# Vi-Sri/CerebralSignalNetworks

Measured on AMD Instinct MI355X. Metric: EEG-segments/sec training (128ch x 500, hidden=768), higher is better.
Workload: dtype bf16

## Files before the change

### cerebralsignalnetworks_amd/cabi.py

```python
import ctypes
import os

import torch

_HERE = os.path.dirname(os.path.abspath(__file__))
LIB_PATH = os.environ.get("CSN_LIB_PATH") or os.path.join(_HERE, "lib", "libcsn_hip.so")

CSN_F32, CSN_BF16 = 0, 1
STATUS_TIMEOUT, STATUS_NONFINITE, STATUS_STALE_SLOT = 1, 2, 4
ABI_VERSION = 6
LSTM_STATE = 0x100
LSTM_DROPOUT = 0x200
LSTM_REVERSE = 0x400
GRAD_OVERWRITE, GRAD_ACCUMULATE = 0, 1
SEG_DECAYED, SEG_SCALED = 1, 2

_c_void_p, _c_int, _c_i64, _c_size_t, _c_float = (ctypes.c_void_p, ctypes.c_int, ctypes.c_int64,
                                                  ctypes.c_size_t, ctypes.c_float)
_c_double = ctypes.c_double


class LstmDesc(ctypes.Structure):
    _fields_ = [("B", ctypes.c_int32), ("T", ctypes.c_int32), ("I", ctypes.c_int32),
                ("H", ctypes.c_int32), ("L", ctypes.c_int32), ("dtype", ctypes.c_int32)]
# ... 160 lines not shown
        _check(load().csn_eeg_bandpass_znorm(_ptr(x), B, C, T, sos.ctypes.data_as(ctypes.POINTER(ctypes.c_double)),
                                             sos.shape[0], int(ddof), _ptr(y), _dt(out_dtype), int(time_major), _stream()))
    return y


def _stream_rows(x_bct):
    B, C, T = x_bct.shape
    if not (x_bct.stride(2) == 1 and x_bct.stride(0) == C * x_bct.stride(1) and x_bct.stride(1) >= T):
        x_bct = x_bct.contiguous()
    return x_bct, x_bct.stride(1)


def _stream_state(t, name, shape, dtype):
    if t is None:
        return
    _need_cuda(t)
    if t.dtype != dtype or tuple(t.shape) != tuple(shape) or not t.is_contiguous():
        raise CsnError(f"eeg_bandpass_stream: {name} must be a contiguous {dtype} tensor of shape {tuple(shape)}, "
                       f"got {t.dtype} {tuple(t.shape)}")


def eeg_bandpass_stream(x_bct, sos, state_in=None, state_out=None, mean=None, inv_std=None, out_dtype=torch.float32,
                        time_major=False):
    import numpy as np
    _need_cuda(x_bct)
    if x_bct.dtype != torch.float32:
        raise CsnError("eeg_bandpass_stream expects float32 input")
    if x_bct.dim() != 3:
        raise CsnError(f"eeg_bandpass_stream expects x[B,C,T], got shape {tuple(x_bct.shape)}")
    x, row_stride = _stream_rows(x_bct)
    B, C, T = x.shape
    sos = np.ascontiguousarray(np.asarray(sos, dtype=np.float64).reshape(-1, 6)) if sos is not None else np.zeros((0, 6))
    nsec = sos.shape[0]
    if (mean is None) != (inv_std is None):
        raise CsnError("eeg_bandpass_stream: mean and inv_std are given together or not at all")
    _stream_state(state_in, "state_in", (B, C, nsec, 2), torch.float64)
    _stream_state(mean, "mean", (C,), torch.float32)
    _stream_state(inv_std, "inv_std", (C,), torch.float32)
    if state_out is None:
        state_out = torch.empty((B, C, nsec, 2), dtype=torch.float64, device=x.device)
    _stream_state(state_out, "state_out", (B, C, nsec, 2), torch.float64)
    y = torch.empty((T, B, C) if time_major else (B, T, C), dtype=out_dtype, device=x.device)
    with torch.cuda.device(x.device):
        _check(load().csn_eeg_bandpass_stream(_ptr(x), row_stride, B, C, T, sos.ctypes.data_as(ctypes.POINTER(ctypes.c_double)),
                                              nsec, _ptr(state_in), _ptr(state_out), _ptr(mean), _ptr(inv_std), _ptr(y),
                                              _dt(out_dtype), int(time_major), _stream()))
    return y, state_out


def eeg_bandpass_stream_path(x_bct, nsec):
    x, row_stride = _stream_rows(x_bct)
    B, C, T = x.shape
    return load().csn_eeg_bandpass_stream_path(_ptr(x), row_stride, C, T, int(nsec))


def eeg_filtfilt(x_stc, sos):
    import numpy as np
    _need_cuda(x_stc)
    x = x_stc.float().contiguous()
    S, T, C = x.shape
    sos = np.ascontiguousarray(np.asarray(sos, dtype=np.float64).reshape(-1, 6))
    lib = load()
    scratch = torch.empty(max(1, lib.csn_eeg_filtfilt_scratch_bytes(S, T, C, sos.shape[0])), dtype=torch.uint8,
                          device=x.device)
    y = torch.empty_like(x)
    with torch.cuda.device(x.device):
        _check(lib.csn_eeg_filtfilt(_ptr(x), S, T, C, sos.ctypes.data_as(ctypes.POINTER(ctypes.c_double)), sos.shape[0],
                                    _ptr(y), _ptr(scratch), _stream()))
    return y


def gemm_nt(a, bt, bias=None, out_dtype=torch.float32, out=None, accumulate=False):
    _need_cuda(a, bt)
    a, bt = a.contiguous(), bt.contiguous()
    M, K = a.shape
    N = bt.shape[0]
    assert bt.shape[1] == K and a.dtype == bt.dtype
    c = out if out is not None else torch.empty((M, N), dtype=out_dtype, device=a.device)
    _check(load().csn_gemm_nt(_ptr(a), _ptr(bt), _ptr(bias), _ptr(c), M, N, K, _dt(a.dtype), _dt(c.dtype),
                              int(accumulate), _stream()))
    return c


def gemm_tn(a_km, b_kn):
    _need_cuda(a_km, b_kn)
    a, b = a_km.contiguous(), b_kn.contiguous()
    K, M = a.shape
    N = b.shape[1]
    assert b.shape[0] == K and a.dtype == b.dtype
    lib = load()
    scratch = torch.empty(max(1, lib.csn_gemm_tn_scratch_bytes(M, N, K)), dtype=torch.uint8, device=a.device)
    c = torch.empty((M, N), dtype=torch.float32, device=a.device)
    _check(lib.csn_gemm_tn(_ptr(a), _ptr(b), _ptr(c), M, N, K, _dt(a.dtype), _ptr(scratch), _stream()))
    return c


def lstm_cell_forward(h_prev, w_hh, xproj, c_prev, want_gates=True):
    _need_cuda(w_hh, xproj)
    B, G = xproj.shape
    H = G // 4
    dt = w_hh.dtype
    gates = torch.empty((B, G), dtype=dt, device=xproj.device) if want_gates else None
    c_out = torch.empty((B, H), dtype=torch.float32, device=xproj.device)
    h_out = torch.empty((B, H), dtype=dt, device=xproj.device)
    _check(load().csn_lstm_cell_forward(_ptr(h_prev), _ptr(w_hh), _ptr(xproj), G, _ptr(c_prev), _ptr(gates),
                                        _ptr(c_out), _ptr(h_out), B, H, _dt(dt), _stream()))
    return h_out, c_out, gates


def lstm_cell_backward(dgates_next, w_hh_t, dy, gates, c, c_prev, dc_carry):
    _need_cuda(gates, c, dc_carry)
    B, G = gates.shape
    H = G // 4
    out = torch.empty_like(gates)
    _check(load().csn_lstm_cell_backward(_ptr(dgates_next), _ptr(w_hh_t), _ptr(dy), H, _ptr(gates), _ptr(c),
                                         _ptr(c_prev), _ptr(dc_carry), _ptr(out), B, H, _dt(gates.dtype), _stream()))
    return out


def _ptr_array(tensors):
    arr = (ctypes.c_void_p * len(tensors))()
    for i, t in enumerate(tensors):
        arr[i] = t.data_ptr()
    return arr


class LstmPlan:

    def __init__(self, B, T, I, H, L, dtype, device, training=True, state=False, dropout=False, reverse=False):
        self.desc = LstmDesc(B, T, I, H, L, _dt(dtype))
        self.training = bool(training)
        self.state = bool(state)
        self.dropout = bool(dropout)
        self.reverse = bool(reverse)
        self._io = (0, 0, False)
        self._views = None
        self.device = torch.device(device)
        lib = load()
        handle = _c_void_p()
        with torch.cuda.device(self.device):
            _check(lib.csn_lstm_plan_create(ctypes.byref(self.desc), int(self.training) | (LSTM_STATE if self.state else 0) |
                                            (LSTM_DROPOUT if self.dropout else 0) | (LSTM_REVERSE if self.reverse else 0),
                                            ctypes.byref(handle)))
        self._plan = handle
        nbytes = lib.csn_lstm_plan_workspace_bytes(self._plan)
        self.workspace = torch.empty(nbytes + 256, dtype=torch.uint8, device=self.device)
        off = (-self.workspace.data_ptr()) % 256
        self._ws_ptr = ctypes.c_void_p(self.workspace.data_ptr() + off)
        self.busy = False
        with torch.cuda.device(self.device):
            _check(lib.csn_lstm_workspace_init(self._plan, self._ws_ptr, _stream()))

    def __del__(self):
        plan, self._plan = getattr(self, "_plan", None), None
        if plan and _lib is not None:
            _lib.csn_lstm_plan_destroy(plan)

    def key(self):
        d = self.desc
        return ((d.B, d.T, d.I, d.H, d.L, d.dtype, self.training) + ((True,) if self.state else ()) +
                (("dropout plan",) if self.dropout else ()) + (("reverse plan",) if self.reverse else ()))

    def path(self):
        return load().csn_lstm_plan_path(self._plan)

    def kernel_names(self):
# ... 416 lines not shown
```

### cerebralsignalnetworks_amd/csrc/csn_common.h

```cpp
#pragma once
#include <hip/hip_runtime.h>
#include <stdint.h>
#include <stdio.h>
#include <stdlib.h>
#include <atomic>
#include <string>

#include "../../include/csn_hip.h"

namespace csn {

typedef __bf16 bf16_t;
typedef __attribute__((ext_vector_type(8))) __bf16 bf16x8;
typedef __attribute__((ext_vector_type(4))) __bf16 bf16x4;
typedef __attribute__((ext_vector_type(4))) float f32x4;
typedef __attribute__((ext_vector_type(4))) short s16x4;

void set_error(const std::string& msg);
int fail(int status, const char* fmt, ...);

#define CSN_HIP_CHECK(expr)                                                              \
  do {                                                                                   \
    hipError_t _e = (expr);                                                              \
    if (_e != hipSuccess)                                                                \
      return ::csn::fail(CSN_ERR_HIP, "%s failed: %s (%s:%d)", #expr, hipGetErrorString(_e), \
                         __FILE__, __LINE__);                                            \
  } while (0)

#define CSN_LAUNCH_CHECK()                                                               \
  do {                                                                                   \
    hipError_t _e = hipGetLastError();                                                   \
    if (_e != hipSuccess)                                                                \
      return ::csn::fail(CSN_ERR_HIP, "kernel launch failed: %s (%s:%d)",                \
                         hipGetErrorString(_e), __FILE__, __LINE__);                     \
  } while (0)

#define CSN_REQUIRE(cond, ...)                                                           \
  do {                                                                                   \
    if (!(cond)) return ::csn::fail(CSN_ERR_INVALID_ARGUMENT, __VA_ARGS__);              \
  } while (0)

struct Options {
  bool cell_v1, no_persist, no_persist_bwd, persist_streams, no_xcd_local, no_rotate, no_fuse_x, no_beside,
      no_side_stream, fwd_ksplit, fwd_nsplit, fwd_flags, bwd_flags, dpoll_no_hint, fwd_hint, gemm_no_dma, gemm_no_256, gemm_generic, tn_no_tr, tn_no_stagger, filter_v1, tags_no_rearm, gemm_no_192, no_half_tiles;
  int chunk;
  int tn_stages;
};
static inline Options options_from_env() {
  auto on = [](const char* name) { return getenv(name) != nullptr; };
  auto num = [](const char* name, int dflt) {
    const char* e = getenv(name);
    return e ? atoi(e) : dflt;
  };
  Options o{};
  o.cell_v1 = on("CSN_CELL_V1");
  o.no_persist = on("CSN_NO_PERSIST");
  o.no_persist_bwd = on("CSN_NO_PERSIST_BWD");
  o.persist_streams = on("CSN_PERSIST_STREAMS");
  o.no_xcd_local = on("CSN_NO_XCD_LOCAL");
  o.no_rotate = on("CSN_NO_ROTATE");
  o.no_fuse_x = on("CSN_NO_FUSE_X");
  o.no_beside = on("CSN_NO_BESIDE");
  o.no_half_tiles = on("CSN_NO_HALF_TILES");
  o.no_side_stream = on("CSN_NO_SIDE_STREAM");
  o.fwd_ksplit = on("CSN_FWD_KSPLIT");
  o.fwd_nsplit = on("CSN_FWD_NSPLIT");
  o.fwd_flags = on("CSN_FWD_FLAGS");
  o.bwd_flags = on("CSN_BWD_FLAGS");
  o.dpoll_no_hint = on("CSN_DPOLL_NO_HINT");
  o.fwd_hint = on("CSN_FWD_HINT");
  o.tn_no_stagger = on("CSN_TN_NO_STAGGER");
  o.gemm_no_dma = on("CSN_GEMM_NO_DMA");
  o.gemm_no_256 = on("CSN_GEMM_NO_256");
  o.gemm_no_192 = on("CSN_GEMM_NO_192");
  o.gemm_generic = on("CSN_GEMM_GENERIC");
  o.tn_no_tr = on("CSN_TN_NO_TR");
  o.filter_v1 = on("CSN_FILTER_V1");
#ifdef CSN_SLAB_TAGS
  o.tags_no_rearm = on("CSN_TAGS_NO_REARM");
#endif
  o.chunk = num("CSN_LSTM_CHUNK", 32);
  if (o.chunk < 1) o.chunk = 1;
  o.tn_stages = num("CSN_TN_STAGES", 4);
  return o;
}

static inline hipStream_t as_stream(csnStream_t s) { return reinterpret_cast<hipStream_t>(s); }
template <auto Kernel>
static int ensure_dyn_lds(int bytes) {
  static std::atomic<unsigned> done{0u};
  int dev = 0;
  CSN_HIP_CHECK(hipGetDevice(&dev));
  const unsigned bit = 1u << (dev & 31);
  if ((done.load(std::memory_order_acquire) & bit) == 0u) {
    CSN_HIP_CHECK(hipFuncSetAttribute(reinterpret_cast<const void*>(Kernel), hipFuncAttributeMaxDynamicSharedMemorySize, bytes));
    done.fetch_or(bit, std::memory_order_release);
  }
  return CSN_OK;
}

static inline size_t align_up(size_t v, size_t a) { return (v + a - 1) / a * a; }
static inline size_t dtype_size(int dtype) { return dtype == CSN_BF16 ? 2 : 4; }

__device__ __forceinline__ float to_f32(float v) { return v; }
__device__ __forceinline__ float to_f32(bf16_t v) { return (float)v; }
template <typename T> __device__ __forceinline__ T from_f32(float v);
template <> __device__ __forceinline__ float from_f32<float>(float v) { return v; }
template <> __device__ __forceinline__ bf16_t from_f32<bf16_t>(float v) { return (bf16_t)v; }

__device__ __forceinline__ float sigmoid_f32(float x) { return 1.0f / (1.0f + expf(-x)); }
__device__ __forceinline__ float tanh_f32(float x) { return tanhf(x); }

struct CellFwdOne {
  const void* h_prev; const void* w_hh; const float* xproj; int64_t xproj_ld; const float* c_prev;
  void* gates_out; float* c_out; void* h_out;
};
struct CellFwdBatch { CellFwdOne p[4]; };
struct CellBwdOne {
  const void* dg_next; const void* w_hh_t; const float* dy; int64_t dy_ld; const void* gates; const float* c;
  const float* c_prev; float* dc_carry; void* dg_out;
};
struct CellBwdBatch { CellBwdOne p[4]; };
struct CellMask {
  const int* lengths;
  int t[4];
};
struct CellNoMask {};
template <bool MASK> struct CellMaskArg { typedef CellNoMask type; };
template <> struct CellMaskArg<true> { typedef CellMask type; };
int launch_cell_fwd_batch(const CellFwdBatch& b, int np, int B, int H, int dtype, hipStream_t st);
int launch_cell_bwd_batch(const CellBwdBatch& b, int np, int B, int H, int dtype, hipStream_t st,
                          const CellMask* mask = nullptr);

int launch_cast_strided(const float* src, int64_t s0, int64_t s1, int64_t n0, int64_t n1, int64_t n2,
                        void* dst, int dtype, hipStream_t st, const int* len = nullptr, int rev = 0,
                        const int* vrow = nullptr, const int* vt0 = nullptr);
int launch_transpose_cast(const float* src, int64_t R, int64_t C, void* dst, int dtype, hipStream_t st);
int launch_cast(const float* src, void* dst, int64_t n, int dtype, hipStream_t st);
int launch_upcast(const void* src, int dtype, float* dst, int64_t n, hipStream_t st);
int launch_add_vec(const float* a, const float* b, float* out, int64_t n, hipStream_t st);
int launch_reduce_slabs(const float* slabs, int64_t stride, int S, float* out, float* out2, int64_t n, int accumulate,
                        hipStream_t st);
size_t colsum_scratch_bytes(int64_t N);
int launch_colsum(const void* X, int64_t R, int64_t N, int dtype, float* out, float* out2, int accumulate, void* scratch,
                  hipStream_t st);
int colsum_chunks();
int launch_colsum_partial(const void* X, int64_t R, int64_t N, int dtype, void* scratch, hipStream_t st);
int launch_gemm_tn_slabs(const void* A, const void* B, float* slabs, int64_t M, int64_t N, int64_t K, int dtype,
                         hipStream_t st, int* S_out, float* colsum, int* colsum_done, const Options& opt);
int gemm_nt(const void* A, const void* Bt, const float* bias, void* C, int64_t M, int64_t N, int64_t K, int dtype,
            int out_dtype, int accumulate, hipStream_t st, const Options& opt);
size_t gemm_tn_scratch_bytes(int64_t M, int64_t N, int64_t K, const Options& opt);

}
```

### cerebralsignalnetworks_amd/csrc/gemm.hip

```cpp
#include "csn_common.h"
#include "lstm_cell_common.h"

namespace csn {

template <typename T>
__global__ void __launch_bounds__(256)
gemm_generic_kernel(const T* __restrict__ A, int64_t sam, int64_t sak, const T* __restrict__ Bm, int64_t sbk,
                    int64_t sbn, const float* __restrict__ bias, void* __restrict__ Cv, int64_t ldc, int64_t M,
                    int64_t N, int64_t K, int out_bf16, int accumulate, int64_t k_per_split, int64_t slab_stride) {
  __shared__ float As[16][64 + 1];
  __shared__ float Bs[16][64 + 1];
  const int tid = threadIdx.x, lane = tid & 63, wave = tid >> 6;
  const int wm = wave >> 1, wn = wave & 1;
  const int64_t m0 = (int64_t)blockIdx.y * 64, n0 = (int64_t)blockIdx.x * 64;
  const int64_t kbeg = (int64_t)blockIdx.z * k_per_split;
  const int64_t kend = (kbeg + k_per_split < K) ? kbeg + k_per_split : K;
  const bool a_kfast = (sak == 1), b_kfast = (sbk == 1);

  f32x4 acc[2][2];
#pragma unroll
  for (int i = 0; i < 2; ++i)
#pragma unroll
    for (int j = 0; j < 2; ++j) acc[i][j] = (f32x4){0.f, 0.f, 0.f, 0.f};

// ... 713 lines not shown
  const int nrot_ = (int)(lid % (unsigned)nk);
#else
  const int nrot_ = 0;
#endif
  auto kpos = [&](int kt) { const int k = kt + nrot_; return (int64_t)(k >= nk ? k - nk : k) * 64; };
  auto issue_a = [&](int kt) {
    char* a_s = smem + (kt % 3) * 32768;
#pragma unroll
    for (int i = 0; i < 4; ++i) glds16(a_src[i] + kpos(kt), a_s + (8 * i + wave) * 1024);
  };
  auto issue_b = [&](int kt) {
    char* b_s = smem + kBBase + (kt % 2) * kBStage;
#pragma unroll
    for (int i = 0; i < NBI; ++i) glds16(b_src[i] + kpos(kt), b_s + (8 * i + wave) * 1024);
  };

  const unsigned sw = (unsigned)((lane & 15) >> 1);
  const unsigned a_base = (unsigned)((wm * 64 + (lane & 15)) * 128) + ((((unsigned)lane >> 4) ^ sw) << 4);
  const unsigned b_base = kBBase + (unsigned)((wn * (BN / 2) + (lane & 15)) * 128) + ((((unsigned)lane >> 4) ^ sw) << 4);

  f32x4 acc[4][NBF];
#pragma unroll
  for (int i = 0; i < 4; ++i)
#pragma unroll
    for (int j = 0; j < NBF; ++j) acc[i][j] = (f32x4){0.f, 0.f, 0.f, 0.f};

  issue_a(0);
  issue_b(0);
  if (nk > 1) issue_a(1);
  for (int kt = 0; kt < nk; ++kt) {
    if (kt + 1 < nk) asm volatile("s_waitcnt vmcnt(4)" ::: "memory");
    else asm volatile("s_waitcnt vmcnt(0)" ::: "memory");
    __builtin_amdgcn_s_barrier();
    if (kt + 1 < nk) issue_b(kt + 1);
    if (kt + 2 < nk) issue_a(kt + 2);
    const unsigned sa = (unsigned)(kt % 3) * 32768u, sb = (unsigned)(kt % 2) * kBStage;
#pragma unroll
    for (int kk = 0; kk < 2; ++kk) {
      const unsigned xo = kk ? 64u : 0u;
      bf16x8 af[4], bfr[NBF];
#pragma unroll
      for (int j = 0; j < NBF; ++j) bfr[j] = lds_read_b128(((b_base ^ xo) + sb) + j * 2048u);
#pragma unroll
      for (int i = 0; i < 4; ++i) af[i] = lds_read_b128(((a_base ^ xo) + sa) + i * 2048u);
#pragma unroll
      for (int i = 0; i < 4; ++i) {
        if (i == 0) asm volatile("s_waitcnt lgkmcnt(3)" ::: "memory");
        else if (i == 1) asm volatile("s_waitcnt lgkmcnt(2)" ::: "memory");
        else if (i == 2) asm volatile("s_waitcnt lgkmcnt(1)" ::: "memory");
        else asm volatile("s_waitcnt lgkmcnt(0)" ::: "memory");
        __builtin_amdgcn_sched_barrier(0);
#pragma unroll
        for (int j = 0; j < NBF; ++j)
          acc[i][j] = __builtin_amdgcn_mfma_f32_16x16x32_bf16(bfr[j], af[i], acc[i][j], 0, 0, 0);
        __builtin_amdgcn_sched_barrier(0);
      }
    }
  }

#pragma unroll
  for (int i = 0; i < 4; ++i) {
    const int64_t m = m0 + wm * 64 + i * 16 + (lane & 15);
    if (m >= M) continue;
#pragma unroll
    for (int j = 0; j < NBF; ++j) {
      const int64_t n = n0 + wn * (BN / 2) + j * 16 + (lane >> 4) * 4;
      f32x4 v = acc[i][j];
      if (bias) v += *reinterpret_cast<const f32x4*>(bias + n);
#if defined(CSN_NT_ABL) && CSN_NT_ABL == 1
      if (v[0] == v[0]) continue;
#endif
      if constexpr (sizeof(OutT) == 4) {
        f32x4* dst = reinterpret_cast<f32x4*>((float*)C + m * N + n);
        if (accumulate) v += *dst;
        *dst = v;
      } else {
        *reinterpret_cast<bf16x4*>((bf16_t*)C + m * N + n) = (bf16x4){(bf16_t)v[0], (bf16_t)v[1], (bf16_t)v[2], (bf16_t)v[3]};
      }
    }
  }
  }
}

__device__ __forceinline__ int tn256_lds_off(int krow, int col) {
  const int sw = (krow & 3) | (((krow >> 3) & 1) << 2);
  return krow * 512 + ((((col >> 4) ^ sw) << 4) + (col & 15)) * 2;
}
__device__ __forceinline__ bf16x8 tn256_load_frag(const char* tile, int mbase, int lane) {
  const int g = lane >> 4, i = lane & 15, q = i >> 2, p = i & 3;
  union { s16x4 s[2]; bf16x8 b; } u;
  u.s[0] = __builtin_amdgcn_ds_read_tr16_b64_v4i16(
      (__attribute__((address_space(3))) s16x4*)(tile + tn256_lds_off(8 * g + q, mbase + 4 * p)));
  u.s[1] = __builtin_amdgcn_ds_read_tr16_b64_v4i16(
      (__attribute__((address_space(3))) s16x4*)(tile + tn256_lds_off(8 * g + 4 + q, mbase + 4 * p)));
  return u.b;
}

__device__ __forceinline__ bf16x8 tr_read_pair(unsigned addr) {
  union { s16x4 s[2]; bf16x8 b; } u;
  asm volatile("ds_read_b64_tr_b16 %0, %1" : "=v"(u.s[0]) : "v"(addr) : "memory");
  asm volatile("ds_read_b64_tr_b16 %0, %1 offset:2048" : "=v"(u.s[1]) : "v"(addr) : "memory");
  return u.b;
}

template <int NSTAGE, bool COLSUM>
__global__ void __launch_bounds__(512)
gemm_tn_256_kernel(const bf16_t* __restrict__ A, const bf16_t* __restrict__ Bm, float* __restrict__ slabs,
                   int64_t M, int64_t N, int64_t K, int64_t k_per_split, float* __restrict__ colsum) {
  extern __shared__ __attribute__((aligned(1024))) char smem[];
  const int tid = threadIdx.x, lane = tid & 63, wave = tid >> 6;
  const int wm = wave >> 2, wn = wave & 3;
  const unsigned ntn = (unsigned)((N + 255) / 256), ntm = (unsigned)((M + 255) / 256);
  const unsigned lid = xcd_remap(blockIdx.x, gridDim.x);
  const unsigned zsplit = lid / (ntm * ntn), rem = lid % (ntm * ntn);
  const int64_t m0 = (int64_t)(rem / ntn) * 256, n0 = (int64_t)(rem % ntn) * 256;
  const int64_t kbeg = (int64_t)zsplit * k_per_split;
  const int64_t kend = (kbeg + k_per_split < K) ? kbeg + k_per_split : K;
  const int nh = kend > kbeg ? (int)((kend - kbeg) / 32) : 0;

  const bf16_t* a_src[2];
  const bf16_t* b_src[2];
#pragma unroll
  for (int i = 0; i < 2; ++i) {
    const int kr = 2 * (8 * i + wave) + (lane >> 5);
    const int c = lane & 31;
    const int sw = (kr & 3) | (((kr >> 3) & 1) << 2);
    const int col = (((c >> 1) ^ sw) << 4) + (c & 1) * 8;
    int64_t am = m0 + col, bn = n0 + col;
    am = am + 8 <= M ? am : M - 8;
    bn = bn + 8 <= N ? bn : N - 8;
    a_src[i] = A + (kbeg + kr) * M + am;
    b_src[i] = Bm + (kbeg + kr) * N + bn;
  }
#if defined(CSN_TN_ROT)
  const int rot_ = nh > CSN_TN_ROT ? (int)(rem % (unsigned)(CSN_TN_ROT)) : 0;
#endif
  auto issue = [&](int h) {
    char* a_s = smem + (h % NSTAGE) * 32768;
    char* b_s = a_s + 16384;
#if defined(CSN_TN_ROT)
    const int hs_ = h + rot_;
    const int64_t hr = hs_ >= nh ? hs_ - nh : hs_;
#else
    const int64_t hr = h;
#endif
#pragma unroll
    for (int i = 0; i < 2; ++i) {
      glds16(a_src[i] + hr * 32 * M, a_s + (8 * i + wave) * 1024);
      glds16(b_src[i] + hr * 32 * N, b_s + (8 * i + wave) * 1024);
    }
  };

  f32x4 acc[8][4];
#pragma unroll
  for (int i = 0; i < 8; ++i)
#pragma unroll
    for (int j = 0; j < 4; ++j) acc[i][j] = (f32x4){0.f, 0.f, 0.f, 0.f};
  const int wn_s = __builtin_amdgcn_readfirstlane(wn);
  const bool do_colsum = COLSUM && colsum != nullptr && n0 == 0;
  const bf16x8 ones = {(bf16_t)1.0f, (bf16_t)1.0f, (bf16_t)1.0f, (bf16_t)1.0f, (bf16_t)1.0f, (bf16_t)1.0f, (bf16_t)1.0f, (bf16_t)1.0f};
  f32x4 acc_cs[2];
  acc_cs[0] = acc_cs[1] = (f32x4){0.f, 0.f, 0.f, 0.f};

  unsigned a_addr[8], b_addr[4];
  {
    const int g = lane >> 4, q = (lane & 15) >> 2, pp = lane & 3;
// ... 243 lines not shown
          if (j == NJ / 4 && 2 * i < NP && more) issue_piece(h + PF, 2 * i);
          if (j == (3 * NJ) / 4 && 2 * i + 1 < NP && more) issue_piece(h + PF, 2 * i + 1);
          __builtin_amdgcn_sched_barrier(0);
#endif
        }
        if constexpr (COLSUM)
          if (own_cs & (1u << i))
            asm volatile("v_mfma_f32_16x16x32_bf16 %0, %1, %2, %0" : "+v"(acc_cs[i]) : "v"(ones), "v"(af[i]));
        __builtin_amdgcn_sched_barrier(0);
      }
      asm volatile("s_waitcnt lgkmcnt(2)" ::: "memory");
      __builtin_amdgcn_sched_barrier(0);
#pragma unroll
      for (int j = 0; j < NJ; ++j) {
#pragma unroll
        for (int k = 0; k < 4; ++k) {
          acc[4 + k][j] = __builtin_amdgcn_mfma_f32_16x16x32_bf16(__builtin_bit_cast(bf16x8, bfr[j]), __builtin_bit_cast(bf16x8, af[4 + k]), acc[4 + k][j], 0, 0, 0);
          __builtin_amdgcn_sched_barrier(0);
          if (k == 0) {
            if (j == 0) af[3] = W4_READ_A(3, sbn);
            else bfr[j - 1] = W4_READ_B(j - 1, sbn);
          }
          if (k == 3 && j == NJ - 1) bfr[j] = W4_READ_B(j, sbn);
          __builtin_amdgcn_sched_barrier(0);
        }
        if constexpr (COLSUM)
          if (j < 4 && (own_cs & (16u << j)))
            asm volatile("v_mfma_f32_16x16x32_bf16 %0, %1, %2, %0" : "+v"(acc_cs[4 + j]) : "v"(ones), "v"(af[4 + j]));
        __builtin_amdgcn_sched_barrier(0);
      }
    }
    asm volatile("s_waitcnt lgkmcnt(0)" ::: "memory");
  }
#undef W4_READ_A
#undef W4_READ_B

  if (COLSUM && (lane >> 4) == 0) {
#pragma unroll
    for (int e = 0; e < 8; ++e) {
      const int64_t m = m0 + wm * 128 + e * 16 + (lane & 15);
      if ((own_cs & (1u << e)) && m < M) colsum[(int64_t)zsplit * M + m] = acc_cs[e][0];
    }
  }

  float* C = slabs + (int64_t)zsplit * M * N;
#pragma unroll
  for (int i = 0; i < 8; ++i) {
    const int64_t m = m0 + wm * 128 + i * 16 + (lane & 15);
    if (m >= M) continue;
#pragma unroll
    for (int j = 0; j < NJ; ++j) {
      const int64_t n = n0 + wn * (BN / 2) + j * 16 + (lane >> 4) * 4;
      if (n + 3 < N && (N & 3) == 0) {
        *reinterpret_cast<float4*>(C + m * N + n) = make_float4(acc[i][j][0], acc[i][j][1], acc[i][j][2], acc[i][j][3]);
      } else {
        for (int r = 0; r < 4; ++r)
          if (n + r < N) C[m * N + n + r] = acc[i][j][r];
      }
    }
  }
}

static int tn_splits(int64_t M, int64_t N, int64_t K) {
  const int64_t tiles = ((M + 127) / 128) * ((N + 127) / 128);
  int64_t s = (1024 + tiles - 1) / tiles;
  const int64_t max_by_k = (K + 511) / 512;
  if (s > max_by_k) s = max_by_k;
  if (s < 1) s = 1;
  if (s > 64) s = 64;
  return (int)s;
}
static bool tn_use_256(int64_t M, int64_t N, int64_t K, const Options& opt) {
  return M >= 256 && N >= 128 && K % 64 == 0 && K >= 8192 && !opt.gemm_no_dma && !opt.gemm_no_256;
}
static int tn_splits_256(int64_t M, int64_t N, int64_t K) {
  const int64_t tiles = ((M + 255) / 256) * ((N + 255) / 256);
  int64_t s = 256 / tiles;
  const int64_t max_by_k = K / 2048;
  if (s > max_by_k) s = max_by_k;
  if (s < 1) s = 1;
  if (s > 64) s = 64;
  return (int)s;
}

int gemm_nt(const void* A, const void* Bt, const float* bias, void* C, int64_t M, int64_t N, int64_t K, int dtype,
            int out_dtype, int accumulate, hipStream_t st, const Options& opt) {
  CSN_REQUIRE(A && Bt && C, "csn_gemm_nt: null pointer");
  CSN_REQUIRE(M > 0 && N > 0 && K > 0, "csn_gemm_nt: bad shape M=%lld N=%lld K=%lld", (long long)M, (long long)N,
              (long long)K);
  CSN_REQUIRE(dtype == CSN_F32 || dtype == CSN_BF16, "csn_gemm_nt: bad dtype %d", dtype);
  CSN_REQUIRE(out_dtype == CSN_F32 || out_dtype == CSN_BF16, "csn_gemm_nt: bad out_dtype %d", out_dtype);
  CSN_REQUIRE(!(accumulate && out_dtype != CSN_F32), "csn_gemm_nt: accumulate needs a float32 C");
  const bool fast = dtype == CSN_BF16 && (K % 8 == 0) && (N % 4 == 0) &&
                    ((reinterpret_cast<uintptr_t>(A) | reinterpret_cast<uintptr_t>(Bt) |
                      reinterpret_cast<uintptr_t>(C) | reinterpret_cast<uintptr_t>(bias)) & 15) == 0 &&
                    !opt.gemm_generic;
  if (!fast)
    return launch_generic(A, K, 1, Bt, 1, K, bias, C, N, M, N, K, dtype, out_dtype, accumulate, 1, 0, st);
  if (K % 64 == 0 && K >= 128 && M >= 256 && !opt.gemm_no_dma && !opt.gemm_no_256 && !opt.gemm_no_192) {
    auto fills = [&](int bn) {
      if (N % bn != 0) return false;
      const int64_t t = (N / bn) * ((M + 255) / 256), rounds = (t + 255) / 256;
      return t >= 256 && t * 10 >= rounds * 256 * 9;
    };
    const int bn = fills(256) ? 256 : (fills(192) ? 192 : 0);
    if (bn != 0) {
      const int lds = 3 * 32768 + 2 * bn * 128;
      dim3 gridw((unsigned)((N / bn) * ((M + 255) / 256)));
      if (bn == 256) {
        if (int rc = ensure_dyn_lds<&gemm_nt_wide_kernel<bf16_t, 256>>(lds)) return rc;
        if (int rc = ensure_dyn_lds<&gemm_nt_wide_kernel<float, 256>>(lds)) return rc;
        if (out_dtype == CSN_BF16)
          gemm_nt_wide_kernel<bf16_t, 256><<<gridw, 512, lds, st>>>((const bf16_t*)A, (const bf16_t*)Bt, bias, (bf16_t*)C, M, N, K, 0);
        else
          gemm_nt_wide_kernel<float, 256><<<gridw, 512, lds, st>>>((const bf16_t*)A, (const bf16_t*)Bt, bias, (float*)C, M, N, K, accumulate);
      } else {
        if (int rc = ensure_dyn_lds<&gemm_nt_wide_kernel<bf16_t, 192>>(lds)) return rc;
        if (int rc = ensure_dyn_lds<&gemm_nt_wide_kernel<float, 192>>(lds)) return rc;
        if (out_dtype == CSN_BF16)
          gemm_nt_wide_kernel<bf16_t, 192><<<gridw, 512, lds, st>>>((const bf16_t*)A, (const bf16_t*)Bt, bias, (bf16_t*)C, M, N, K, 0);
        else
          gemm_nt_wide_kernel<float, 192><<<gridw, 512, lds, st>>>((const bf16_t*)A, (const bf16_t*)Bt, bias, (float*)C, M, N, K, accumulate);
      }
      CSN_LAUNCH_CHECK();
      return CSN_OK;
    }
  }
  if (K % 64 == 0 && K >= 256 && M >= 256 && N >= 1024 && !opt.gemm_no_dma && !opt.gemm_no_256) {
    if (int rc = ensure_dyn_lds<&gemm_nt_256_kernel<bf16_t, 3>>(3 * 49152)) return rc;
    if (int rc = ensure_dyn_lds<&gemm_nt_256_kernel<float, 3>>(3 * 49152)) return rc;
    dim3 grid256((unsigned)(((N + 127) / 128) * ((M + 255) / 256)));
    if (out_dtype == CSN_BF16)
      gemm_nt_256_kernel<bf16_t, 3><<<grid256, 512, 3 * 49152, st>>>((const bf16_t*)A, (const bf16_t*)Bt, bias, (bf16_t*)C, M, N, K, 0);
    else
      gemm_nt_256_kernel<float, 3><<<grid256, 512, 3 * 49152, st>>>((const bf16_t*)A, (const bf16_t*)Bt, bias, (float*)C, M, N, K, accumulate);
    CSN_LAUNCH_CHECK();
    return CSN_OK;
  }
  dim3 grid((unsigned)(((N + 127) / 128) * ((M + 127) / 128)));
  if (K % 64 == 0 && !opt.gemm_no_dma) {
    if (int rc = ensure_dyn_lds<&gemm_nt_dma_kernel<bf16_t>>(98304)) return rc;
    if (int rc = ensure_dyn_lds<&gemm_nt_dma_kernel<float>>(98304)) return rc;
    if (out_dtype == CSN_BF16)
      gemm_nt_dma_kernel<bf16_t><<<grid, 256, 65536, st>>>((const bf16_t*)A, (const bf16_t*)Bt, bias, (bf16_t*)C, M, N, K, 0);
    else
      gemm_nt_dma_kernel<float><<<grid, 256, 65536, st>>>((const bf16_t*)A, (const bf16_t*)Bt, bias, (float*)C, M, N, K, accumulate);
    CSN_LAUNCH_CHECK();
    return CSN_OK;
  }
  if (out_dtype == CSN_BF16)
    gemm_nt_bf16_kernel<bf16_t, 1><<<grid, 256, 32768, st>>>((const bf16_t*)A, (const bf16_t*)Bt, bias, (bf16_t*)C, M, N, K, 0);
  else
    gemm_nt_bf16_kernel<float, 1><<<grid, 256, 32768, st>>>((const bf16_t*)A, (const bf16_t*)Bt, bias, (float*)C, M, N, K, accumulate);
  CSN_LAUNCH_CHECK();
  return CSN_OK;
}

}

using namespace csn;

extern "C" int csn_gemm_nt(const void* A, const void* Bt, const float* bias, void* C, int64_t M, int64_t N, int64_t K,
                           int dtype, int out_dtype, int accumulate, csnStream_t stream) {
  return gemm_nt(A, Bt, bias, C, M, N, K, dtype, out_dtype, accumulate, as_stream(stream), options_from_env());
}

namespace csn {
size_t gemm_tn_scratch_bytes(int64_t M, int64_t N, int64_t K, const Options& opt) {
  if (M <= 0 || N <= 0 || K <= 0) return 0;
  const int a = tn_splits(M, N, K), b = tn_use_256(M, N, K, opt) ? tn_splits_256(M, N, K) : 0;
  return (size_t)(a > b ? a : b) * (size_t)M * (size_t)N * sizeof(float);
}
}

extern "C" size_t csn_gemm_tn_scratch_bytes(int64_t M, int64_t N, int64_t K) {
  return gemm_tn_scratch_bytes(M, N, K, options_from_env());
}

namespace csn {
int launch_gemm_tn_slabs(const void* A, const void* B, float* slabs, int64_t M, int64_t N, int64_t K, int dtype,
                         hipStream_t st, int* S_out, float* colsum, int* colsum_done, const Options& opt) {
  if (colsum_done) *colsum_done = 0;
  const bool aligned16 = ((reinterpret_cast<uintptr_t>(A) | reinterpret_cast<uintptr_t>(B)) & 15) == 0;
  if (dtype == CSN_BF16 && (M % 8 == 0) && (N % 8 == 0) && aligned16 && tn_use_256(M, N, K, opt)) {
    const int S2 = tn_splits_256(M, N, K);
    int64_t kper2 = (K + S2 - 1) / S2;
    kper2 = (kper2 + 63) / 64 * 64;
    *S_out = S2;
    if (int rc = ensure_dyn_lds<&gemm_tn_256_kernel<5, false>>(5 * 32768)) return rc;
    if (int rc = ensure_dyn_lds<&gemm_tn_256_kernel<4, false>>(4 * 32768)) return rc;
    if (int rc = ensure_dyn_lds<&gemm_tn_256_kernel<3, false>>(3 * 32768)) return rc;
    if (int rc = ensure_dyn_lds<&gemm_tn_256_kernel<4, true>>(4 * 32768)) return rc;
    dim3 grid((unsigned)(((N + 255) / 256) * ((M + 255) / 256) * S2));
    const int nst = opt.tn_stages;
    const bf16_t* Ab = (const bf16_t*)A;
    const bf16_t* Bb = (const bf16_t*)B;
    if (!opt.tn_no_stagger && nst == 4) {
      constexpr int NS = CSN_TN_W4_NSTAGE, PF = CSN_TN_W4_PF;
      if (N <= 128) {
        constexpr int lds = NS * (16384 + 8192);
        if (int rc = ensure_dyn_lds<&gemm_tn_256w4_kernel<NS, PF, false, 128>>(lds)) return rc;
        if (int rc = ensure_dyn_lds<&gemm_tn_256w4_kernel<NS, PF, true, 128>>(lds)) return rc;
        if (colsum) gemm_tn_256w4_kernel<NS, PF, true, 128><<<grid, 256, lds, st>>>(Ab, Bb, slabs, M, N, K, kper2, colsum);
        else gemm_tn_256w4_kernel<NS, PF, false, 128><<<grid, 256, lds, st>>>(Ab, Bb, slabs, M, N, K, kper2, nullptr);
      } else {
        constexpr int lds = NS * 32768;
        if (int rc = ensure_dyn_lds<&gemm_tn_256w4_kernel<NS, PF, false, 256>>(lds)) return rc;
        if (int rc = ensure_dyn_lds<&gemm_tn_256w4_kernel<NS, PF, true, 256>>(lds)) return rc;
        if (colsum) gemm_tn_256w4_kernel<NS, PF, true, 256><<<grid, 256, lds, st>>>(Ab, Bb, slabs, M, N, K, kper2, colsum);
        else gemm_tn_256w4_kernel<NS, PF, false, 256><<<grid, 256, lds, st>>>(Ab, Bb, slabs, M, N, K, kper2, nullptr);
      }
    } else if (colsum) gemm_tn_256_kernel<4, true><<<grid, 512, 4 * 32768, st>>>(Ab, Bb, slabs, M, N, K, kper2, colsum);
    else if (nst == 3) gemm_tn_256_kernel<3, false><<<grid, 512, 3 * 32768, st>>>(Ab, Bb, slabs, M, N, K, kper2, nullptr);
    else if (nst == 5) gemm_tn_256_kernel<5, false><<<grid, 512, 5 * 32768, st>>>(Ab, Bb, slabs, M, N, K, kper2, nullptr);
    else gemm_tn_256_kernel<4, false><<<grid, 512, 4 * 32768, st>>>(Ab, Bb, slabs, M, N, K, kper2, nullptr);
    if (colsum && colsum_done) *colsum_done = 1;
    CSN_LAUNCH_CHECK();
    return CSN_OK;
  }
  const int S = tn_splits(M, N, K);
  int64_t kper = (K + S - 1) / S;
  kper = (kper + 63) / 64 * 64;
  *S_out = S;
  const bool fast = dtype == CSN_BF16 && (M % 8 == 0) && (N % 8 == 0) &&
                    ((reinterpret_cast<uintptr_t>(A) | reinterpret_cast<uintptr_t>(B)) & 15) == 0 &&
                    !opt.gemm_generic;
  if (fast) {
    dim3 grid((unsigned)(((N + 127) / 128) * ((M + 127) / 128) * S));
    if (opt.tn_no_tr)
      gemm_tn_bf16_kernel<false><<<grid, 256, 0, st>>>((const bf16_t*)A, (const bf16_t*)B, slabs, M, N, K, kper);
    else
      gemm_tn_bf16_kernel<true><<<grid, 256, 0, st>>>((const bf16_t*)A, (const bf16_t*)B, slabs, M, N, K, kper);
    CSN_LAUNCH_CHECK();
    return CSN_OK;
  }
  return launch_generic(A, 1, M, B, N, 1, nullptr, slabs, N, M, N, K, dtype, CSN_F32, 0, S, M * N, st);
}
}

extern "C" int csn_gemm_tn(const void* A, const void* B, float* C, int64_t M, int64_t N, int64_t K, int dtype,
                           void* scratch, csnStream_t stream) {
  CSN_REQUIRE(A && B && C && scratch, "csn_gemm_tn: null pointer");
  CSN_REQUIRE(M > 0 && N > 0 && K > 0, "csn_gemm_tn: bad shape");
  CSN_REQUIRE(dtype == CSN_F32 || dtype == CSN_BF16, "csn_gemm_tn: bad dtype %d", dtype);
  hipStream_t st = as_stream(stream);
  int S = 1;
  if (int rc = launch_gemm_tn_slabs(A, B, (float*)scratch, M, N, K, dtype, st, &S, nullptr, nullptr, options_from_env())) return rc;
  return launch_reduce_slabs((const float*)scratch, M * N, S, C, nullptr, M * N, 0, st);
}
```

Baseline: 27010.

## Add 4-wave 256x192 NT GEMM kernel with two workgroups per CU

Adds a new bf16 NT GEMM kernel for the 192-wide tile case that uses 256 threads (4 waves) with 128x96 per-wave tiles, an A ring buffer of depth 3 and a double-buffered B stage. It uses swizzled LDS, hand-scheduled ds_read and MFMA interleaving, and async global-to-LDS loads. LDS is capped at 80KB so two workgroups can fit per CU. The aim is better occupancy and overlap than the 512-thread wide kernel on the 192-column path. The cost is high register pressure from 48 accumulators per lane. It also requires 32-bit byte offsets, which is guarded by a fit check.

```diff
diff --git a/cerebralsignalnetworks_amd/cabi.py b/cerebralsignalnetworks_amd/cabi.py
--- a/cerebralsignalnetworks_amd/cabi.py
+++ b/cerebralsignalnetworks_amd/cabi.py
@@ -266,6 +266,18 @@
     return c
 
 
+def gemm_nt_w4_offsets_fit(M, N, K):
+    fn = load().csn_gemm_nt_w4_offsets_fit
+    fn.restype, fn.argtypes = _c_int, [_c_i64, _c_i64, _c_i64]
+    return bool(fn(M, N, K))
+
+
+def gemm_nt_w4_lds_bytes():
+    fn = load().csn_gemm_nt_w4_lds_bytes
+    fn.restype, fn.argtypes = _c_int, []
+    return int(fn())
+
+
 def gemm_tn(a_km, b_kn):
     _need_cuda(a_km, b_kn)
     a, b = a_km.contiguous(), b_kn.contiguous()
diff --git a/cerebralsignalnetworks_amd/csrc/csn_common.h b/cerebralsignalnetworks_amd/csrc/csn_common.h
--- a/cerebralsignalnetworks_amd/csrc/csn_common.h
+++ b/cerebralsignalnetworks_amd/csrc/csn_common.h
@@ -42,7 +42,7 @@
 
 struct Options {
   bool cell_v1, no_persist, no_persist_bwd, persist_streams, no_xcd_local, no_rotate, no_fuse_x, no_beside,
-      no_side_stream, fwd_ksplit, fwd_nsplit, fwd_flags, bwd_flags, dpoll_no_hint, fwd_hint, gemm_no_dma, gemm_no_256, gemm_generic, tn_no_tr, tn_no_stagger, filter_v1, tags_no_rearm, gemm_no_192, no_half_tiles;
+      no_side_stream, fwd_ksplit, fwd_nsplit, fwd_flags, bwd_flags, dpoll_no_hint, fwd_hint, gemm_no_dma, gemm_no_256, gemm_generic, tn_no_tr, tn_no_stagger, filter_v1, tags_no_rearm, gemm_no_192, no_half_tiles, nt_no_w4;
   int chunk;
   int tn_stages;
 };
@@ -73,6 +73,7 @@
   o.gemm_no_dma = on("CSN_GEMM_NO_DMA");
   o.gemm_no_256 = on("CSN_GEMM_NO_256");
   o.gemm_no_192 = on("CSN_GEMM_NO_192");
+  o.nt_no_w4 = on("CSN_NT_NO_W4");
   o.gemm_generic = on("CSN_GEMM_GENERIC");
   o.tn_no_tr = on("CSN_TN_NO_TR");
   o.filter_v1 = on("CSN_FILTER_V1");
diff --git a/cerebralsignalnetworks_amd/csrc/gemm.hip b/cerebralsignalnetworks_amd/csrc/gemm.hip
--- a/cerebralsignalnetworks_amd/csrc/gemm.hip
+++ b/cerebralsignalnetworks_amd/csrc/gemm.hip
@@ -819,6 +819,120 @@
   }
 }
 
+#ifndef CSN_NT_W4_NA
+#define CSN_NT_W4_NA 3
+#endif
+__device__ __forceinline__ int nt64_sw(int row) {
+  const int g = (row >> 2) & 3;
+  return (((g ^ (g >> 1)) & 1) << 1) | (g >> 1);
+}
+template <typename OutT, int NA>
+__global__ void __launch_bounds__(256, 2)
+gemm_nt_w4_kernel(const bf16_t* __restrict__ A, const bf16_t* __restrict__ Bt, const float* __restrict__ bias,
+                  OutT* __restrict__ C, int64_t M, int64_t N, int64_t K, int accumulate) {
+  static_assert(NA == 2 || NA == 3, "A ring depth");
+  constexpr unsigned kAStage = 16384u, kBStage = 12288u, kBBase = NA * kAStage;
+  static_assert(kBBase + 2 * kBStage <= 81920u, "two workgroups per CU");
+  extern __shared__ __attribute__((aligned(1024))) char smem[];
+  const int tid = threadIdx.x, lane = tid & 63;
+  const int wave = __builtin_amdgcn_readfirstlane(tid >> 6);
+  const int wm = wave >> 1, wn = wave & 1;
+  const unsigned ntn = (unsigned)(N / 192);
+  const unsigned lid = xcd_remap(blockIdx.x, gridDim.x);
+  const int64_t m0 = (int64_t)(lid / ntn) * 256, n0 = (int64_t)(lid % ntn) * 192;
+  const int nk = __builtin_amdgcn_readfirstlane((int)(K / 32));
+
+  unsigned a_off[4], b_off[3];
+#pragma unroll
+  for (int i = 0; i < 4; ++i) {
+    const int row = (4 * i + wave) * 16 + (lane >> 2);
+    const int ch = (lane & 3) ^ nt64_sw(row);
+    int64_t am = m0 + row;
+    am = am < M ? am : M - 1;
+    a_off[i] = (unsigned)((am * K + ch * 8) * 2);
+  }
+#pragma unroll
+  for (int i = 0; i < 3; ++i) {
+    const int row = (4 * i + wave) * 16 + (lane >> 2);
+    const int ch = (lane & 3) ^ nt64_sw(row);
+    b_off[i] = (unsigned)(((n0 + row) * K + ch * 8) * 2);
+  }
+  auto issue_a = [&](int kt, int i) {
+    glds16(reinterpret_cast<const char*>(A + (int64_t)kt * 32) + a_off[i], smem + (unsigned)(kt % NA) * kAStage + (4 * i + wave) * 1024);
+  };
+  auto issue_b = [&](int kt, int i) {
+    glds16(reinterpret_cast<const char*>(Bt + (int64_t)kt * 32) + b_off[i], smem + kBBase + (unsigned)(kt & 1) * kBStage + (4 * i + wave) * 1024);
+  };
+
+  const unsigned frag = (unsigned)((lane & 15) * 64) + ((((unsigned)lane >> 4) ^ (unsigned)nt64_sw(lane & 15)) << 4);
+  const unsigned a_base = (unsigned)(wm * 128 * 64) + frag;
+  const unsigned b_base = kBBase + (unsigned)(wn * 96 * 64) + frag;
+#define W4_READ(addr, off) ({ bf16x8 v_; asm volatile("ds_read_b128 %0, %1 offset:%2" : "=v"(v_) : "v"(addr), "n"(off) : "memory"); v_; })
+
+  f32x4 acc[8][6];
+#pragma unroll
+  for (int i = 0; i < 8; ++i)
+#pragma unroll
+    for (int j = 0; j < 6; ++j) acc[i][j] = (f32x4){0.f, 0.f, 0.f, 0.f};
+
+#pragma unroll
+  for (int i = 0; i < 4; ++i) issue_a(0, i);
+#pragma unroll
+  for (int i = 0; i < 3; ++i) issue_b(0, i);
+  if (NA == 3 && nk > 1) {
+#pragma unroll
+    for (int i = 0; i < 4; ++i) issue_a(1, i);
+  }
+  for (int kt = 0; kt < nk; ++kt) {
+    if (NA == 3 && kt + 1 < nk) asm volatile("s_waitcnt vmcnt(4)" ::: "memory");
+    else asm volatile("s_waitcnt vmcnt(0)" ::: "memory");
+    __builtin_amdgcn_s_barrier();
+    const bool more_b = kt + 1 < nk, more_a = kt + NA - 1 < nk;
+    const unsigned aa = a_base + (unsigned)(kt % NA) * kAStage, ba = b_base + (unsigned)(kt & 1) * kBStage;
+    bf16x8 af[2], bfr[6];
+#pragma unroll
+    for (int j = 0; j < 6; ++j) bfr[j] = W4_READ(ba, j * 1024);
+    af[0] = W4_READ(aa, 0);
+#pragma unroll
+    for (int i = 0; i < 8; ++i) {
+      if (i < 7) af[(i + 1) & 1] = W4_READ(aa, (i + 1) * 1024);
+      if (i < 7) asm volatile("s_waitcnt lgkmcnt(1)" ::: "memory");
+      else asm volatile("s_waitcnt lgkmcnt(0)" ::: "memory");
+      __builtin_amdgcn_sched_barrier(0);
+#pragma unroll
+      for (int j = 0; j < 6; ++j) {
+        acc[i][j] = __builtin_amdgcn_mfma_f32_16x16x32_bf16(bfr[j], af[i & 1], acc[i][j], 0, 0, 0);
+        __builtin_amdgcn_sched_barrier(0);
+        if (j == 1) {
+          if (i < 3) { if (more_b) issue_b(kt + 1, i); }
+          else if (i < 7) { if (more_a) issue_a(kt + NA - 1, i - 3); }
+          __builtin_amdgcn_sched_barrier(0);
+        }
+      }
+    }
+  }
+#undef W4_READ
+
+#pragma unroll
+  for (int i = 0; i < 8; ++i) {
+    const int64_t m = m0 + wm * 128 + i * 16 + (lane & 15);
+    if (m >= M) continue;
+#pragma unroll
+    for (int j = 0; j < 6; ++j) {
+      const int64_t n = n0 + wn * 96 + j * 16 + (lane >> 4) * 4;
+      f32x4 v = acc[i][j];
+      if (bias) v += *reinterpret_cast<const f32x4*>(bias + n);
+      if constexpr (sizeof(OutT) == 4) {
+        f32x4* dst = reinterpret_cast<f32x4*>((float*)C + m * N + n);
+        if (accumulate) v += *dst;
+        *dst = v;
+      } else {
+        *reinterpret_cast<bf16x4*>((bf16_t*)C + m * N + n) = (bf16x4){(bf16_t)v[0], (bf16_t)v[1], (bf16_t)v[2], (bf16_t)v[3]};
+      }
+    }
+  }
+}
+
 __device__ __forceinline__ int tn256_lds_off(int krow, int col) {
   const int sw = (krow & 3) | (((krow >> 3) & 1) << 2);
   return krow * 512 + ((((col >> 4) ^ sw) << 4) + (col & 15)) * 2;
@@ -1228,6 +1342,13 @@
   if (s > 64) s = 64;
   return (int)s;
 }
+
+static bool nt_w4_offsets_fit(int64_t M, int64_t N, int64_t K) {
+  const int64_t lim = (int64_t)1 << 31;
+  return M <= lim / K && N <= lim / K && M * K < lim && N * K < lim;
+}
+static constexpr int kNtW4LdsBytes = CSN_NT_W4_NA * 16384 + 2 * 12288;
+static_assert(kNtW4LdsBytes <= 81920, "two workgroups of gemm_nt_w4_kernel per CU");
 
 int gemm_nt(const void* A, const void* Bt, const float* bias, void* C, int64_t M, int64_t N, int64_t K, int dtype,
             int out_dtype, int accumulate, hipStream_t st, const Options& opt) {
@@ -1260,6 +1381,13 @@
           gemm_nt_wide_kernel<bf16_t, 256><<<gridw, 512, lds, st>>>((const bf16_t*)A, (const bf16_t*)Bt, bias, (bf16_t*)C, M, N, K, 0);
         else
           gemm_nt_wide_kernel<float, 256><<<gridw, 512, lds, st>>>((const bf16_t*)A, (const bf16_t*)Bt, bias, (float*)C, M, N, K, accumulate);
+      } else if (!opt.nt_no_w4 && nt_w4_offsets_fit(M, N, K)) {
+        if (int rc = ensure_dyn_lds<&gemm_nt_w4_kernel<bf16_t, CSN_NT_W4_NA>>(kNtW4LdsBytes)) return rc;
+        if (int rc = ensure_dyn_lds<&gemm_nt_w4_kernel<float, CSN_NT_W4_NA>>(kNtW4LdsBytes)) return rc;
+        if (out_dtype == CSN_BF16)
+          gemm_nt_w4_kernel<bf16_t, CSN_NT_W4_NA><<<gridw, 256, kNtW4LdsBytes, st>>>((const bf16_t*)A, (const bf16_t*)Bt, bias, (bf16_t*)C, M, N, K, 0);
+        else
+          gemm_nt_w4_kernel<float, CSN_NT_W4_NA><<<gridw, 256, kNtW4LdsBytes, st>>>((const bf16_t*)A, (const bf16_t*)Bt, bias, (float*)C, M, N, K, accumulate);
       } else {
         if (int rc = ensure_dyn_lds<&gemm_nt_wide_kernel<bf16_t, 192>>(lds)) return rc;
         if (int rc = ensure_dyn_lds<&gemm_nt_wide_kernel<float, 192>>(lds)) return rc;
@@ -1318,6 +1446,11 @@
   return (size_t)(a > b ? a : b) * (size_t)M * (size_t)N * sizeof(float);
 }
 }
+
+extern "C" int csn_gemm_nt_w4_offsets_fit(int64_t M, int64_t N, int64_t K) {
+  return M > 0 && N > 0 && K > 0 && nt_w4_offsets_fit(M, N, K) ? 1 : 0;
+}
+extern "C" int csn_gemm_nt_w4_lds_bytes(void) { return kNtW4LdsBytes; }
 
 extern "C" size_t csn_gemm_tn_scratch_bytes(int64_t M, int64_t N, int64_t K) {
   return gemm_tn_scratch_bytes(M, N, K, options_from_env());
```

Result: faster. 27300 (median of 6 runs) (+1.0%).
